# drtconway/zotmer

Hardware: AMD Instinct MI355X
Metric: Gk-mers/sec kmerize k=25 on synthetic 150bp FASTQ; achieved HBM GB/s fraction (higher is better)
Workload: dtype u64

## Files before the change

include/zotk.h:

```cpp
#ifndef ZOTK_H
#define ZOTK_H

#include <stdint.h>

#ifdef __cplusplus
extern "C" {
#endif

#define ZK_OK 0
#define ZK_EINVAL (-1)
#define ZK_ENOMEM (-2)
#define ZK_EHIP (-3)
#define ZK_ENOSPC (-4)
#define ZK_EOVERFLOW (-5)
#define ZK_EINTERNAL (-6)
#define ZK_ERANGE (-7)

typedef struct zk_ctx zk_ctx;

zk_ctx* zk_create(int device, uint64_t workspace_bytes);
void zk_destroy(zk_ctx* ctx);
const char* zk_last_error(zk_ctx* ctx);
int zk_set_stream(zk_ctx* ctx, void* hip_stream);
void* zk_get_stream(zk_ctx* ctx);
// ... 11 lines not shown
int zk_upload_async(zk_ctx* ctx, void* d_dst, const void* src, uint64_t bytes);

#define ZK_TUNE_SORT_VARIANT 1
#define ZK_TUNE_PAIRS_VARIANT 2
#define ZK_TUNE_SHORT_SORT 3
#define ZK_TUNE_XCD_GROUP 5
#define ZK_TUNE_SIDE_DIV 4
#define ZK_TUNE_EARLY_COLLAPSE 7
#define ZK_TUNE_PACKED_PAIRS 8
#define ZK_TUNE_WIDE_TILES 9
#define ZK_TUNE_STREAM_PASS 10
#define ZK_TUNE_STREAM_RANGES 11
#define ZK_TUNE_TAG_WORDS 12
#define ZK_TUNE_DEDUPE_VARIANT 13
#define ZK_TUNE_DEDUPE_LIMIT 14
#define ZK_TUNE_DEDUPE_BITS 15
#define ZK_TUNE_COMM_CHUNK 6
#define ZK_TUNE_TAG_PASS 17
#define ZK_TUNE_KWAY 18
#define ZK_TUNE_TILE_SORT 19
#define ZK_TUNE_STRAND_BLOCKS 20
#define ZK_TUNE_COMM_SELF_LOOP 16
int zk_tune(zk_ctx* ctx, int what, int value);

#define ZK_PROF_HIST_STREAM 1
#define ZK_PROF_HIST_ARRAY 2
#define ZK_PROF_PASS_STREAM 3
#define ZK_PROF_PASS_KEYS 4
#define ZK_PROF_PASS_PAIRS 5
#define ZK_PROF_RLE 6
#define ZK_PROF_UNION 7
#define ZK_PROF_SELECT 8
#define ZK_PROF_MIRROR 9
#define ZK_PROF_INTERSECT 10
#define ZK_PROF_COUNT_HIST 11
#define ZK_PROF_PASS_PACKED 12
#define ZK_PROF_SAMPLE 13
#define ZK_PROF_TILE_SORT 14
#define ZK_PROF_CAPTURE_HITS 15
#define ZK_PROF_PROJECT_SUM 16
#define ZK_PROF_SPECTRUM 17
int zk_debug_buffer(zk_ctx* ctx, void* d_buf);
int zk_profile(zk_ctx* ctx, int enable);
int zk_profile_read(zk_ctx* ctx, int tag, uint64_t* launches, double* total_ms, uint64_t* algorithmic_bytes);


// ... 172 lines not shown
```

zotmer_amd/csrc/context.hip:

```cpp
#include <stdarg.h>
#include <string.h>

#include "internal.hpp"
#include <vector>

namespace zk {

int fail(zk_ctx* c, int code, const char* fmt, ...) {
    char buf[512];
    va_list ap;
    va_start(ap, fmt);
    vsnprintf(buf, sizeof buf, fmt, ap);
    va_end(ap);
    if (c) c->last_error = buf;
    return code;
}

void arena_reset(zk_ctx* c) { c->arena_off = 0; }

int arena_alloc(zk_ctx* c, uint64_t bytes, void** p) {
    const uint64_t need = (bytes + 255) & ~255ull;
    if (c->arena_off + need > c->arena_size) {
        if (c->arena_off != 0)
            return fail(c, ZK_ENOMEM, "workspace too small: %llu bytes in use, %llu more needed, %llu reserved (call zk_reserve)",
// ... 273 lines not shown
    if (what == ZK_TUNE_PAIRS_VARIANT) { c->pairs_variant = value; return ZK_OK; }
    if (what == ZK_TUNE_SHORT_SORT) { c->short_sort = value; return ZK_OK; }
    if (what == ZK_TUNE_SIDE_DIV) { c->side_div = value; return ZK_OK; }
    if (what == ZK_TUNE_WIDE_TILES) { c->wide_tiles = value ? 1 : 0; return ZK_OK; }
    if (what == ZK_TUNE_PACKED_PAIRS) { c->packed_pairs = value ? 1 : 0; return ZK_OK; }
    if (what == ZK_TUNE_EARLY_COLLAPSE) { c->early_collapse = value < 0 ? 0 : (value > 3 ? 3 : value); return ZK_OK; }
    if (what == ZK_TUNE_COMM_SELF_LOOP) { c->comm_self_loop = value ? 1 : 0; return ZK_OK; }
    if (what == ZK_TUNE_COMM_CHUNK) { c->comm_chunk_bytes = value > 0 ? (uint64_t)value : 0; return ZK_OK; }
    if (what == ZK_TUNE_STREAM_PASS) {
#ifdef ZK_PHASES
        c->stream_pass = value < 0 ? 0 : value;
#else
        if (value < 0 || value > 3) return fail(c, ZK_EINVAL, "stream pass variant %d (0, 1, 2 or 3)", value);
        c->stream_pass = value;
#endif
        return ZK_OK;
    }
    if (what == ZK_TUNE_TAG_WORDS) { c->tag_words = value < 0 ? 0 : (value > 2 ? 2 : value); return ZK_OK; }
    if (what == ZK_TUNE_DEDUPE_VARIANT) { c->dedupe_variant = value < 0 ? -1 : (value & 3); return ZK_OK; }
    if (what == ZK_TUNE_KWAY) { c->kway = value < 0 ? 0 : (value > 2 ? 2 : value); return ZK_OK; }
    if (what == ZK_TUNE_TILE_SORT) { c->tile_sort = value ? 1 : 0; return ZK_OK; }
    if (what == ZK_TUNE_TAG_PASS) { c->tag_pass = value ? 1 : 0; return ZK_OK; }
    if (what == ZK_TUNE_DEDUPE_BITS) { c->dedupe_bits = value < 0 ? 0 : value; return ZK_OK; }
    if (what == ZK_TUNE_STRAND_BLOCKS) { c->strand_blocks = value < 0 ? 0 : (value > 3 ? 1 : value); return ZK_OK; }
    if (what == ZK_TUNE_DEDUPE_LIMIT) { c->dedupe_limit = value < 1 ? 1 : (value > 65536 ? 65536 : value); return ZK_OK; }
    if (what == ZK_TUNE_STREAM_RANGES) { c->stream_ranges = value < 0 ? 0 : (value > 4096 ? 4096 : value); return ZK_OK; }
    if (what == ZK_TUNE_XCD_GROUP) {
        if (value < 0 || value > 32 || (value & (value - 1))) return fail(c, ZK_EINVAL, "xcd group must be 0 or a power of two <= 32");
        c->xcd_group = value;
        return ZK_OK;
    }
    return fail(c, ZK_EINVAL, "unknown tuning knob %d", what);
}

int zk_debug_buffer(zk_ctx* c, void* d_buf) {
    if (!c) return ZK_EINVAL;
    enter(c);
    c->dbg = (u64*)d_buf;
    return ZK_OK;
}

int zk_profile(zk_ctx* c, int enable) {
    if (!c) return ZK_EINVAL;
    enter(c);
    ZK_HIP(c, hipStreamSynchronize(c->stream));
    for (auto& r : c->prof) { (void)hipEventDestroy(r.a); (void)hipEventDestroy(r.b); }
    c->prof.clear();
    c->profile = enable != 0;
    return ZK_OK;
}

int zk_profile_read(zk_ctx* c, int tag, uint64_t* launches, double* total_ms, uint64_t* total_bytes) {
    if (!c) return ZK_EINVAL;
    enter(c);
    ZK_HIP(c, hipStreamSynchronize(c->stream));
// ... 83 lines not shown
```

zotmer_amd/csrc/internal.hpp:

```cpp
#pragma once
#include <hip/hip_runtime.h>
#include <stdint.h>
#include <stdio.h>
#include <string>
#include <vector>

#include "../../include/zotk.h"
#include "common.hpp"

struct zk_ctx {
    int device = 0;
    hipStream_t stream = nullptr;
    bool own_stream = false;
    int num_cus = 256;
    int sort_variant = 3;
    int short_sort = 0;
    int packed_pairs = 1;
    int wide_tiles = 1;
    int early_collapse = 1;
    int side_div = 8;
    int pairs_variant = 7;
    int stream_pass = 1;
    int tag_words = 2;
    int dedupe_variant = 0;
    int dedupe_limit = 65536;
    int tag_pass = 0;
    int kway = 1;
    int tile_sort = 1;
    int dedupe_bits = 0;
    int strand_blocks = 1;
    int stream_ranges = 0;

    char* arena = nullptr;
    uint64_t arena_size = 0;
    uint64_t arena_off = 0;

    char* aux = nullptr;
    uint64_t aux_size = 0;

    u64* status = nullptr;
    uint64_t status_words = 0;
    unsigned short* part16 = nullptr;
    uint64_t part16_words = 0;
    u32 epoch = 0;
    u32* d_ticket = nullptr;
    u32* d_xticket = nullptr;
    int num_xcd = 1;
    int xcd_group = 0;
    u32 ticket_base = 0;

    u32* d_err = nullptr;
    u64* d_scalars = nullptr;
// ... 67 lines not shown
                   StreamTags* tags = nullptr; };
int sort_rbits(zk_ctx* c);
PassPlan sort_plan_upper(zk_ctx* c, int key_bits, int lo_bit);
struct MirrorHist { int passes; int shift[4]; int bits[4]; u64* raw; };
int sort_first_bits(zk_ctx* c, int key_bits, int lo_bit);
struct DedupeResult {
    uint64_t n_out = 0;
    uint32_t flags = 0;
    uint32_t n_big = 0;
    u64 *cuts = nullptr, *nwords = nullptr, *incl = nullptr, *big = nullptr, *work = nullptr;
    u32* sub = nullptr;
    uint32_t chunks = 0;
    int pack = 0;
    int tag_bits = 0;
    bool unsorted = false;
};
int dedupe_pass(zk_ctx* c, const u64* keys, uint64_t n, int key_bits, int b, int pack, u64* work, uint64_t cap, DedupeResult* r,
                uint64_t* n_in = nullptr, uint64_t max_chunks = 0, const u32* tags = nullptr, const u64* tag_cuts = nullptr,
                bool unsorted = false);
int dedupe_sort_blocks(zk_ctx* c, DedupeResult& r);
int expand_tags(zk_ctx* c, const u32* tags, const u64* cuts, uint32_t blocks, int tag_bits, u64* keys_out, uint64_t first_block = 0, uint64_t n_blocks = 0);
int dedupe_finish(zk_ctx* c, const DedupeResult& r, u64* out_k, u32* out_c, u64* out_m = nullptr, int K = 0, int gbases = 0,
                  u64** mirror_hist = nullptr, int* mirror_group_bits = nullptr, bool packed_out = false);
int sort_keys_upper_counted(zk_ctx* c, u64* keys, u64* alt, uint64_t n, int key_bits, int lo_bit, u64* counted, u64** result);
int strand_blocks(zk_ctx* c, const DedupeResult& r, u64* keys_buf, uint64_t buf_words, int K, u64* out_k, u32* out_c, uint64_t cap,
                  uint64_t* n_out);
int collapse_pass(zk_ctx* c, const u64* keys, uint64_t n, int shift, int bits, int pack, u64* out, uint64_t cap, uint64_t* n_out,
                  uint64_t max_tiles = 0);
int sort_stream(zk_ctx* c, const StreamSrc& src, u64* buf_a, u64* buf_b, uint64_t cap, uint64_t* n_keys,
                uint64_t acgt[4], u64** result);
struct StreamRows { u32* rows = nullptr; u64* offs = nullptr; u32 ranges = 0, radix = 0; u32* gcodes = nullptr; u16* gvalid = nullptr;
                    u32 strands = 1;
                    bool wide = false; };
int stream_hist(zk_ctx* c, const u8* stream, uint64_t n_bytes, int K, int mode, const PassPlan& plan, u64* ghist, u32 gstride,
                u64* d_acgt, u64* d_n, u64* rec_info, u64* sample, u32 sample_cap, int sample_shift, u64 sample_value, u32* sample_n,
                void* image_room, uint64_t image_room_bytes, StreamRows* out);
struct StreamPlanes { u16* dig; int shift, bits; };
int stream_pass0(zk_ctx* c, uint64_t n_bytes, int K, int mode, int shift, int bits, const u64* ghist0, const StreamRows& rows,
                 uint64_t first_nl, bool uniform, u64* kout, uint64_t n, int variant, const StreamPlanes* planes = nullptr);
int stream_pass1(zk_ctx* c, const u32* tags, const u16* dig, uint64_t n, const u64* ghist0, uint32_t radix0, int bits1, u32* tout, u64* cuts);
int tile_sort_top_bits(uint64_t n, int key_bits, int rbits);
int tile_sort(zk_ctx* c, u64* keys, u32* vals, uint64_t n, int key_bits, int top, bool* declined);
int tile_sort_count(zk_ctx* c, const u64* keys, uint64_t n, int key_bits, int top, u64* uniq, u32* counts, uint64_t cap, uint64_t* n_unique,
                    bool* declined);
int trim(zk_ctx* c, const u64* keys, const void* cnts, int cbits, uint64_t n, u64 lo, u64 hi, u64* ok, void* oc,
         uint64_t cap, uint64_t* n_out);
int project_dedupe(zk_ctx* c, const u64* keys, uint64_t n, int shift, u64* out, uint64_t cap, uint64_t* n_out);
// ... 45 lines not shown
```

zotmer_amd/csrc/pipeline.hip:

```cpp
#include <string.h>

#include <vector>

#include "internal.hpp"

namespace zk {

__global__ void mirror_kernel(const u64* __restrict__ c, const u32* __restrict__ n, u64 m, int K, u64* __restrict__ r,
                              u32* __restrict__ v) {
    for (u64 i = (u64)blockIdx.x * blockDim.x + threadIdx.x; i < m; i += (u64)gridDim.x * blockDim.x) {
        r[i] = revcomp(K, c[i]);
        v[i] = n[i];
    }
}

constexpr int MIRROR_GROUP_BITS = 18;
constexpr int MIRROR_GROUP_BASES = MIRROR_GROUP_BITS / 2;

__global__ void mirror_bounds_kernel(const u64* __restrict__ c, u64 n, int K, int gbits, u64* __restrict__ start) {
    const u32 g = blockIdx.x * blockDim.x + threadIdx.x;
    if (g > (1u << gbits)) return;
    const u64 want = (u64)g << (2 * K - gbits);
    u64 lo = 0, hi = n;
    if (g == (1u << gbits)) lo = n;
// ... 317 lines not shown
        st->n_canonical = 0;
        return rle(c, sorted, n, out_k, out_c, cap, n_out);
    }
    u64* other = (sorted == buf_a) ? buf_b : buf_a;
    u32* cnt = (u32*)other;
    uint64_t uc = 0;
    bool in_aux = false;
    uint64_t max_count = 0;
    bool have_max = false;
    bool canon_packed = false;
    u64 *mwords = nullptr, *malt = nullptr;
    u64* mhist = nullptr;
    int mgroup = MIRROR_GROUP_BITS;
    if (dedupe_bit && n) {
        const int pk = pack_bits_for(K);
        DedupeResult r;
        uint64_t n_in = 0;
        bool done = false;
        const uint64_t nblocks = 1ull << dedupe_bit, per = n / nblocks + 1;
        const u32* tg = stags.written ? (const u32*)sorted : nullptr;
        if (!presampled) ZK_TRY(dedupe_pass(c, sorted, n, 2 * K, dedupe_bit, pk, other, cap_keys, &r, &n_in, (1u << 20) / per + 4, tg, stags.cuts));
        if (presampled || (!(r.flags & 1) && (double)r.n_out <= 0.6 * (double)n_in)) {
            const bool route = !canonical_only && c->packed_pairs && dedupe_bit == MIRROR_GROUP_BITS && 2 * K >= MIRROR_GROUP_BITS + 8 &&
                               (K & 1) && (c->strand_blocks == 1 || c->strand_blocks == 3);
            ZK_TRY(dedupe_pass(c, sorted, n, 2 * K, dedupe_bit, pk, other, cap_keys, &r, nullptr, 0, tg, stags.cuts, route));
            if (!(r.flags & 1)) {
                uc = r.n_out;
                const uint64_t a8 = (8 * uc + 255) & ~255ull, a4 = (4 * uc + 255) & ~255ull;
                const bool want_m = !(r.flags & 2) && !canonical_only && c->packed_pairs && dedupe_bit == MIRROR_GROUP_BITS &&
                                    2 * K >= MIRROR_GROUP_BITS + 8;
                if (want_m && (K & 1) && c->strand_blocks && 2 * a8 <= 8 * cap_keys) {
                    st->n_canonical = uc;
                    return strand_blocks(c, r, sorted, cap_keys, K, out_k, out_c, cap, n_out);
                }
                if (r.unsorted) ZK_TRY(dedupe_sort_blocks(c, r));
                char* aux;
                ZK_TRY(aux_require(c, a8 + a4, &aux));
                ZK_TRY(dedupe_finish(c, r, (u64*)aux, (u32*)(aux + a8), want_m ? sorted : nullptr, K, MIRROR_GROUP_BASES, &mhist, &mgroup, want_m));
                if (want_m) { mwords = sorted; malt = other; canon_packed = true; }
                sorted = (u64*)aux; cnt = (u32*)(aux + a8);
                in_aux = true;
                if (!(r.flags & 2)) { max_count = (1ull << pk) - 1; have_max = true; }
                done = true;
            }
        }
        if (!done) {
            u64* res = nullptr;
// ... 320 lines not shown
```

zotmer_amd/csrc/radix_sort.hip:

```cpp
#include <stdlib.h>
#include "internal.hpp"
#include "encode_tile.hpp"
#include "dedupe.hpp"

namespace zk {

constexpr int MAX_RADIX = 1024;

enum { SRC_ARRAY = 0, SRC_STREAM = 1 };

template <int BLOCK_, int ITEMS_, int RBITS_, int ROUNDS_ = 1, int WPE_ = 1, int SEG_ = 32, bool PIPE_ = false>
struct Cfg {
    static constexpr int BLOCK = BLOCK_, ITEMS = ITEMS_, RBITS = RBITS_, ROUNDS = ROUNDS_, WPE = WPE_, SEG = SEG_;
    static constexpr bool PIPE = PIPE_;
    static_assert(SEG == 0 || (BLOCK * ITEMS < 32768 && (SEG & (SEG - 1)) == 0), "16-bit tile counts");
    static constexpr int TILE = BLOCK * ITEMS, RADIX = 1 << RBITS, NW = BLOCK / 64;
    static constexpr int EXCH = TILE / ROUNDS, IPR = ITEMS / ROUNDS;
    static_assert(ITEMS % ROUNDS == 0, "ROUNDS");
    static constexpr int DPT = (RADIX + BLOCK - 1) / BLOCK;
    static_assert(ITEMS % 2 == 0 && 2 * ITEMS < 256, "ITEMS");
    static_assert(64 * ITEMS < 65536, "per-wave ranks are 16-bit");
    static_assert(RADIX <= MAX_RADIX && RBITS * MAX_PASSES >= 64, "RBITS");
};

// ... 1131 lines not shown
template <class C, bool PAIRS = false>
struct PipeSmem {
    static constexpr bool IMG_FITS = sizeof(TileImage<C::TILE>) <= sizeof(u16) * C::NW * C::RADIX;
    static constexpr int IMG_WORDS = (int)(sizeof(u16) * C::NW * C::RADIX / 8);
    static constexpr int IMG_T = IMG_FITS ? (IMG_WORDS - 3) * 16 : 16;
    u64 exch[C::TILE];
    u32 exv[PAIRS ? C::TILE : 1];
    union {
        u16 cnt[C::NW][C::RADIX];
        TileImage<PipeSmem::IMG_T> img;
    };
    u32 digit_off[C::RADIX];
    u64 gbase[C::RADIX];
    u32 wsum[C::NW];
    u32 ticket;
    u32 total_live;
    u32 abort;
};

template <class C, int SRC, int VAR = 0>
__global__ __launch_bounds__(C::BLOCK, C::WPE) void pass_pipe_kernel(SortArgs a, u32 tiles) {
    constexpr int BLOCK = C::BLOCK, ITEMS = C::ITEMS, RADIX = C::RADIX, NW = C::NW, DPT = C::DPT, TILE = C::TILE;
    constexpr bool PAIRS = VAR == 5 || VAR == 6;
    constexpr bool ATOM = VAR == 3 || VAR == 4 || VAR == 6, TAGS = VAR == 2 || VAR == 3;
    static_assert(!PAIRS || SRC == SRC_ARRAY, "pairs come from arrays");
    static_assert(!ATOM || (SRC == SRC_ARRAY && NW >= 2), "the counters of the adds are the first two rows of the per-wave counters");
    static_assert(C::ROUNDS == 1, "the pipeline parks a whole tile in LDS");
    constexpr int NS = RADIX / 64;
    __shared__ PipeSmem<C, VAR == 5 || VAR == 6> sm;
    static_assert(SRC == SRC_ARRAY || PipeSmem<C>::IMG_FITS, "the tile image lives in the counter area");
    static_assert(SRC == SRC_ARRAY || (ITEMS == 16 && PipeSmem<C>::IMG_WORDS <= 2 * BLOCK), "stream source: 16 consecutive windows per thread");
    const int tid = threadIdx.x, lane = tid & 63, wave = __builtin_amdgcn_readfirstlane(tid >> 6);
    const u32 dmask = (1u << a.bits) - 1u;
    u16* mycnt = sm.cnt[wave];

    if (tid == 0) sm.abort = 0;
    u32* cnt32 = reinterpret_cast<u32*>(&sm.cnt[0][0]);
    if (ATOM && tid < RADIX) cnt32[tid] = 0;
    bool dirty = false;
    const u32 first = take_ticket(a.ticket, &sm.ticket) - a.ticket_base;
    if (first < (u32)NS) {
        constexpr int U = 32;
        __builtin_amdgcn_s_setprio(3);
        u64* carry = sm.exch;
        if (tid < 64) carry[tid] = 0;
        __syncthreads();
        const u64 tag = st_pack(ZK_ST_INCLUSIVE, a.epoch, 0);
// ... 413 lines not shown
    static int launch_pipe(zk_ctx* c, SortArgs a) {
      if constexpr (C::PIPE) {
        const u32 tiles = tiles_for(a, SRC);
        if (tiles == 0) return ZK_OK;
        u32 grid = (u32)c->num_cus * (sizeof(PipeSmem<C>) > 80 * 1024 ? 1 : 2);
        if (grid > tiles) grid = tiles;
        grid += C::RADIX / 64;
        ZK_TRY(lookback_begin(c, (uint64_t)tiles * C::RADIX, grid, &a.epoch, &a.ticket_base));
        ZK_TRY(part16_begin(c, (uint64_t)tiles * C::RADIX, &a.part));
        ZK_HIP(c, hipMemsetAsync(c->d_xticket, 0, 8 * 32 * sizeof(u32), c->stream));
        a.xticket = c->d_xticket;
        a.nx = (c->xcd_group > 0 && c->num_xcd == 8) ? 8u : 1u;
        a.glog = 0;
        while ((1 << (a.glog + 1)) <= c->xcd_group) a.glog++;
        a.status = c->status;
        a.ticket = c->d_ticket;
        a.err = c->d_err;
        a.dbg = c->dbg;
        a.dbg2 = c->dbg ? c->dbg + 8ull * tiles : nullptr;
        prof_begin(c, SRC == SRC_STREAM ? ZK_PROF_PASS_STREAM : (a.prof_tag ? a.prof_tag : ZK_PROF_PASS_KEYS),
                   SRC == SRC_STREAM ? a.n_bytes + 8 * a.n : (a.tags_out ? 12 : 16) * a.n);
        if (SRC == SRC_ARRAY && a.tags_out && a.straddle)
            hipLaunchKernelGGL((pass_pipe_kernel<C, SRC_ARRAY, 3>), dim3(grid), dim3(C::BLOCK), 0, c->stream, a, tiles);
        else if (SRC == SRC_ARRAY && a.straddle)
            hipLaunchKernelGGL((pass_pipe_kernel<C, SRC_ARRAY, 4>), dim3(grid), dim3(C::BLOCK), 0, c->stream, a, tiles);
        else if (SRC == SRC_ARRAY && a.tags_out)
            hipLaunchKernelGGL((pass_pipe_kernel<C, SRC_ARRAY, 2>), dim3(grid), dim3(C::BLOCK), 0, c->stream, a, tiles);
        else if (SRC == SRC_ARRAY && a.prof_tag == ZK_PROF_PASS_PACKED)
            hipLaunchKernelGGL((pass_pipe_kernel<C, SRC, 1>), dim3(grid), dim3(C::BLOCK), 0, c->stream, a, tiles);
        else
            hipLaunchKernelGGL((pass_pipe_kernel<C, SRC, 0>), dim3(grid), dim3(C::BLOCK), 0, c->stream, a, tiles);
        prof_end(c);
        ZK_HIP(c, hipGetLastError());
      }
      return ZK_OK;
    }
    static constexpr bool PIPE_PAIRS = C::PIPE && C::ITEMS <= 8;
    static int launch_pipe_pairs(zk_ctx* c, SortArgs a) {
      if constexpr (PIPE_PAIRS) {
        const u32 tiles = (u32)div_up(a.n, C::TILE);
        if (tiles == 0) return ZK_OK;
        u32 grid = (u32)c->num_cus * (sizeof(PipeSmem<C, true>) > 80 * 1024 ? 1 : 2);
        if (grid > tiles) grid = tiles;
        grid += C::RADIX / 64;
        ZK_TRY(lookback_begin(c, (uint64_t)tiles * C::RADIX, grid, &a.epoch, &a.ticket_base));
        ZK_TRY(part16_begin(c, (uint64_t)tiles * C::RADIX, &a.part));
        ZK_HIP(c, hipMemsetAsync(c->d_xticket, 0, 8 * 32 * sizeof(u32), c->stream));
        a.xticket = c->d_xticket;
        a.nx = 1u;
        a.glog = 0;
        a.status = c->status;
        a.ticket = c->d_ticket;
        a.err = c->d_err;
        a.dbg = nullptr; a.dbg2 = nullptr;
        prof_begin(c, ZK_PROF_PASS_PAIRS, 24 * a.n);
        if (a.straddle) hipLaunchKernelGGL((pass_pipe_kernel<C, SRC_ARRAY, 6>), dim3(grid), dim3(C::BLOCK), 0, c->stream, a, tiles);
        else hipLaunchKernelGGL((pass_pipe_kernel<C, SRC_ARRAY, 5>), dim3(grid), dim3(C::BLOCK), 0, c->stream, a, tiles);
        prof_end(c);
        ZK_HIP(c, hipGetLastError());
      }
      return ZK_OK;
    }
    static u32 keys_pass_tile(zk_ctx* c, uint64_t n) {
        if constexpr (C::PIPE && C::RBITS == 9 && C::BLOCK == 512) { if (c->wide_tiles && n <= WIDE_TILES_MAX_KEYS) return 16384u; }
        return (u32)C::TILE;
    }
    static int launch_keys_pass(zk_ctx* c, const SortArgs& a) {
        if constexpr (C::PIPE && C::RBITS == 9 && C::BLOCK == 512) { if (c->wide_tiles && a.n <= WIDE_TILES_MAX_KEYS) return launch_wide_pass(c, a); }
        if (C::PIPE) return launch_pipe<SRC_ARRAY>(c, a);
        return launch_pass<SRC_ARRAY, false>(c, a);
    }

    template <int SRC>
    static int launch_hist(zk_ctx* c, const SortArgs& src, const PassPlan& plan, u64* ghist, u64* acgt, u64* d_n,
                           u64* sample = nullptr, u32 sample_cap = 0, int sample_shift = 0, u64 sample_value = 0) {
        HistArgs h;
        h.sample = sample; h.sample_cap = sample_cap; h.sample_shift = sample_shift; h.sample_value = sample_value;
        h.sample_n = (u32*)(c->d_scalars + 23);
        if (sample) ZK_HIP(c, hipMemsetAsync(c->d_scalars + 23, 0, sizeof(u64), c->stream));
        h.src = src;
        h.plan = plan;
        h.ghist = ghist;
        h.acgt = acgt;
        h.tiles = tiles_for(src, SRC);
        h.rec_info = nullptr;
        ZK_HIP(c, hipMemsetAsync(ghist, 0, sizeof(u64) * MAX_PASSES * C::RADIX, c->stream));
        if (SRC == SRC_STREAM && src.n_bytes) {
            h.rec_info = c->d_scalars + 20;
            ZK_HIP(c, hipMemsetAsync(h.rec_info, 0, 3 * sizeof(u64), c->stream));
            hipLaunchKernelGGL(first_newline_kernel, dim3(1), dim3(256), 0, c->stream, src.stream, (u64)src.n_bytes, h.rec_info);
        }
        if (acgt) ZK_HIP(c, hipMemsetAsync(acgt, 0, sizeof(u64) * 4, c->stream));
        u32 grid = h.tiles < (u32)(c->num_cus * 8) ? h.tiles : (u32)(c->num_cus * 8);
        if (grid == 0) grid = 1;
        prof_begin(c, SRC == SRC_STREAM ? ZK_PROF_HIST_STREAM : ZK_PROF_HIST_ARRAY, SRC == SRC_STREAM ? src.n_bytes : 8 * src.n);
        if constexpr (SRC == SRC_STREAM && C::ITEMS == 16 && C::BLOCK <= 512) {
            if (src.mode != ZK_KEYS_BOTH) hipLaunchKernelGGL((hist_kernel<C, SRC, true>), dim3(grid), dim3(C::BLOCK), 0, c->stream, h);
            else hipLaunchKernelGGL((hist_kernel<C, SRC, false>), dim3(grid), dim3(C::BLOCK), 0, c->stream, h);
        } else {
            hipLaunchKernelGGL((hist_kernel<C, SRC, false>), dim3(grid), dim3(C::BLOCK), 0, c->stream, h);
        }
        prof_end(c);
        ZK_HIP(c, hipGetLastError());
        hipLaunchKernelGGL(hist_scan_kernel, dim3(1), dim3(256), 0, c->stream, ghist, plan.passes, (int)C::RADIX, d_n);
        ZK_HIP(c, hipGetLastError());
        return ZK_OK;
    }

    static int sort_keys(zk_ctx* c, u64* keys, u64* alt, uint64_t n, int key_bits, u64** result, int lo_bit = 0, int prof_tag = 0,
                         u64* counted = nullptr) {
        PassPlan plan = make_plan(key_bits - lo_bit, C::RBITS, lo_bit);
        u64* ghist = counted;
        if (!counted) ZK_TRY(arena_alloc(c, sizeof(u64) * MAX_PASSES * C::RADIX, (void**)&ghist));
        SortArgs a = {};
        a.kin = keys; a.n = n;
        a.prof_tag = prof_tag;
        if (counted) {
            hipLaunchKernelGGL(hist_scan_kernel, dim3(1), dim3(256), 0, c->stream, ghist, plan.passes, (int)C::RADIX, c->d_scalars + 8);
            ZK_HIP(c, hipGetLastError());
        } else {
            ZK_TRY(launch_hist<SRC_ARRAY>(c, a, plan, ghist, nullptr, c->d_scalars + 8));
        }
        u64* in = keys; u64* out = alt;
        for (int p = 0; p < plan.passes; p++) {
            a.kin = in; a.kout = out; a.shift = plan.shift[p]; a.bits = plan.bits[p];
            a.ghist = ghist + p * C::RADIX;
            ZK_TRY(launch_keys_pass(c, a));
            u64* t = in; in = out; out = t;
        }
        *result = in;
        return ZK_OK;
    }

    static int sort_pairs(zk_ctx* c, u64* keys, u64* alt, u32* vals, u32* valt, uint64_t n, int key_bits, u64** rk, u32** rv,
                          const u64* src_k = nullptr, const u32* src_v = nullptr, int mirror_K = 0, int lo_bit = 0, bool unordered = false) {
        PassPlan plan = make_plan(key_bits - lo_bit, C::RBITS, lo_bit);
        u64* ghist;
        ZK_TRY(arena_alloc(c, sizeof(u64) * MAX_PASSES * C::RADIX, (void**)&ghist));
        SortArgs a = {};
        a.kin = mirror_K ? src_k : keys; a.n = n; a.mirror_K = mirror_K;
        ZK_TRY(launch_hist<SRC_ARRAY>(c, a, plan, ghist, nullptr, c->d_scalars + 8));
        const u64* in = mirror_K ? src_k : keys; const u32* vi = mirror_K ? src_v : vals;
        u64* out = mirror_K ? keys : alt; u32* vo = mirror_K ? vals : valt;
        for (int p = 0; p < plan.passes; p++) {
            a.kin = in; a.kout = out; a.vin = vi; a.vout = vo; a.shift = plan.shift[p]; a.bits = plan.bits[p];
            a.ghist = ghist + p * C::RADIX;
            a.mirror_K = (p == 0) ? mirror_K : 0;
            if constexpr (PIPE_PAIRS) {
                a.straddle = nullptr;
                if (unordered && p <= 1) {
                    const u32 tiles = (u32)div_up(n, C::TILE);
                    u32* bm;
                    ZK_TRY(arena_alloc(c, sizeof(u32) * (tiles / 32 + 1), (void**)&bm));
                    ZK_HIP(c, hipMemsetAsync(bm, 0, sizeof(u32) * (tiles / 32 + 1), c->stream));
                    if (p == 1) {
                        hipLaunchKernelGGL(straddle_kernel, dim3((C::RADIX + 255) / 256), dim3(256), 0, c->stream, (const u64*)(ghist + (p - 1) * C::RADIX),
                                           1u << plan.bits[p - 1], (u32)C::TILE, bm);
                        ZK_HIP(c, hipGetLastError());
                    }
                    a.straddle = bm;
                }
                ZK_TRY(launch_pipe_pairs(c, a));
            } else
            ZK_TRY((launch_pass<SRC_ARRAY, true>(c, a)));
            in = out; vi = vo;
            out = (out == keys) ? alt : keys;
            vo = (vo == vals) ? valt : vals;
        }
        *rk = const_cast<u64*>(in); *rv = const_cast<u32*>(vi);
        return ZK_OK;
    }

    static int sort_stream(zk_ctx* c, const StreamSrc& src, u64* buf_a, u64* buf_b, uint64_t cap, uint64_t* n_keys,
                           uint64_t acgt[4], u64** result) {
        const int top = (src.hi_bit > 0 && src.hi_bit < 2 * src.K) ? src.hi_bit : 2 * src.K;
        PassPlan plan = make_plan(top - src.lo_bit, C::RBITS, src.lo_bit);
        u64* ghist;
        ZK_TRY(arena_alloc(c, sizeof(u64) * MAX_PASSES * C::RADIX, (void**)&ghist));
        SortArgs a = {};
        a.stream = src.stream; a.n_bytes = src.n_bytes; a.K = src.K; a.mode = src.mode;
        u64* d_acgt = c->d_scalars + 0;
        u64* d_n = c->d_scalars + 8;
// ... 74 lines not shown
                    const uint32_t cpr = (uint32_t)((W + 15) / 16);
                    const uint32_t rpt = (C::BLOCK / cpr) / 16 * 16;
                    if (rpt >= 16 && (uint64_t)rpt * rec / 16 + 3 <= (uint64_t)PipeSmem<C>::IMG_WORDS &&
                        (double)rpt * (double)W > 1.02 * (double)C::TILE * (double)W / (double)rec) {
                        a.rec = (u32)rec; a.rpt = rpt; a.cpr = cpr; a.wpr = (u32)W;
                        a.cpr_inv = (u32)(((1ull << 32) + cpr - 1) / cpr);
                    }
                }
            }
            if (src.mode != ZK_KEYS_BOTH) ZK_TRY(launch_pipe<SRC_STREAM>(c, a));
            else ZK_TRY((launch_pass<SRC_STREAM, false>(c, a)));
        } else {
            ZK_TRY((launch_pass<SRC_STREAM, false>(c, a)));
        }
        u64* in = buf_a; u64* out = buf_b;
        a.rec = 0;
        const bool tags = src.tags && C::PIPE && plan.passes == 2 && plan.shift[0] <= 32 && src.mode == ZK_KEYS_CANONICAL;
        for (int p = 1; p < plan.passes; p++) {
            a.kin = in; a.kout = out; a.shift = plan.shift[p]; a.bits = plan.bits[p];
            a.ghist = ghist + p * C::RADIX;
            a.tags_out = (tags && p == plan.passes - 1) ? 1 : 0;
            a.straddle = nullptr;
            if ((a.tags_out || p == 1) && c->tag_words >= 2 && C::PIPE) {
                const u32 tile = keys_pass_tile(c, n), tiles = (u32)div_up(n, tile);
                u32* bm;
                ZK_TRY(arena_alloc(c, sizeof(u32) * (tiles / 32 + 1), (void**)&bm));
                ZK_HIP(c, hipMemsetAsync(bm, 0, sizeof(u32) * (tiles / 32 + 1), c->stream));
                hipLaunchKernelGGL(straddle_kernel, dim3((C::RADIX + 255) / 256), dim3(256), 0, c->stream, (const u64*)(ghist + (p - 1) * C::RADIX),
                                   1u << plan.bits[p - 1], tile, bm);
                ZK_HIP(c, hipGetLastError());
                a.straddle = bm;
            }
#ifdef ZK_PHASES
            if (const char* e = getenv("ZK_LOCAL_PASS")) a.dbg_local = atoi(e);
#endif
            ZK_TRY(launch_keys_pass(c, a));
#ifdef ZK_PHASES
            if (a.dbg_local) { *n_keys = 0; return ZK_OK; }
#endif
            if (a.tags_out) {
                const u32 tile = keys_pass_tile(c, n), tiles = (u32)div_up(n, tile);
                const uint64_t blocks = 1ull << (plan.bits[0] + plan.bits[1]);
                u64* cuts;
                ZK_TRY(arena_alloc(c, sizeof(u64) * (blocks + 1), (void**)&cuts));
                hipLaunchKernelGGL(tag_cuts_kernel, dim3(1u << plan.bits[0]), dim3(512), 0, c->stream, (const u64*)in, (u64)n, (const u64*)ghist,
                                   (const u64*)(ghist + C::RADIX), (const u64*)c->status, (u32)C::RADIX, tile, tiles, plan.shift[1], plan.bits[1],
                                   plan.bits[0], cuts);
                ZK_HIP(c, hipGetLastError());
                src.tags->cuts = cuts; src.tags->blocks = (uint32_t)blocks; src.tags->written = true;
            }
            u64* t = in; in = out; out = t;
        }
        *result = in;
// ... 48 lines not shown

int sort_pairs(zk_ctx* c, u64* keys, u64* alt, u32* vals, u32* valt, uint64_t n, int key_bits, u64** rk, u32** rv) {
    *rk = keys; *rv = vals;
    if (n == 0) return ZK_OK;
    const int top = c->tile_sort ? tile_sort_top_bits(n, key_bits, sort_pairs_rbits(c)) : 0;
    if (top) {
        u64* k1 = nullptr; u32* v1 = nullptr;
        bool declined = false;
        ZK_TRY(sort_pairs_upper(c, keys, alt, vals, valt, n, key_bits, key_bits - top, &k1, &v1));
        ZK_TRY(tile_sort(c, k1, v1, n, key_bits, top, &declined));
        *rk = k1; *rv = v1;
        if (!declined) return ZK_OK;
        return sort_pairs_lsd(c, k1, k1 == keys ? alt : keys, v1, v1 == vals ? valt : vals, n, key_bits, rk, rv);
    }
    return sort_pairs_lsd(c, keys, alt, vals, valt, n, key_bits, rk, rv);
}

int sort_keys_upper(zk_ctx* c, u64* keys, u64* alt, uint64_t n, int key_bits, int lo_bit, u64** result, int prof_tag) {
    *result = keys;
    if (n == 0 || lo_bit >= key_bits) return ZK_OK;
    ZK_SORT_DISPATCH(c, sort_keys(c, keys, alt, n, key_bits, result, lo_bit, prof_tag));
}

int sort_keys_upper_counted(zk_ctx* c, u64* keys, u64* alt, uint64_t n, int key_bits, int lo_bit, u64* counted, u64** result) {
    *result = keys;
    if (n == 0 || lo_bit >= key_bits) return ZK_OK;
    return Sorter<V3>::sort_keys(c, keys, alt, n, key_bits, result, lo_bit, ZK_PROF_PASS_PACKED, counted);
}

int sort_pairs_upper(zk_ctx* c, u64* keys, u64* alt, u32* vals, u32* valt, uint64_t n, int key_bits, int lo_bit, u64** rk, u32** rv) {
    *rk = keys; *rv = vals;
    if (n == 0) return ZK_OK;
    if (c->pairs_variant == 7) return Sorter<V7>::sort_pairs(c, keys, alt, vals, valt, n, key_bits, rk, rv, nullptr, nullptr, 0, lo_bit);
    ZK_SORT_DISPATCH_V(c->pairs_variant, sort_pairs(c, keys, alt, vals, valt, n, key_bits, rk, rv, nullptr, nullptr, 0, lo_bit));
}

int sort_pairs_mirrored(zk_ctx* c, const u64* src_k, const u32* src_v, u64* keys, u64* alt, u32* vals, u32* valt, uint64_t n, int K,
                        u64** rk, u32** rv, int lo_bit) {
    *rk = keys; *rv = vals;
    if (n == 0) return ZK_OK;
    if (c->pairs_variant == 7) return Sorter<V7>::sort_pairs(c, keys, alt, vals, valt, n, 2 * K, rk, rv, src_k, src_v, K, lo_bit, true);
    ZK_SORT_DISPATCH_V(c->pairs_variant, sort_pairs(c, keys, alt, vals, valt, n, 2 * K, rk, rv, src_k, src_v, K, lo_bit));
}
int sort_pairs_rbits(zk_ctx* c) { return (c->pairs_variant == 0 || c->pairs_variant == 1 || c->pairs_variant == 5) ? 8 : 9; }

PassPlan sort_plan_upper(zk_ctx* c, int key_bits, int lo_bit) { return make_plan(key_bits - lo_bit, sort_rbits(c), lo_bit); }

int sort_rbits(zk_ctx* c) {
    switch (c->sort_variant) { case 0: case 1: case 5: return 8; default: return 9; }
}
// ... 208 lines not shown
```

zotmer_amd/csrc/strand_blocks.hip:

```cpp
#include "tile_group.hpp"

namespace zk {

constexpr int SB_ITEMS = 16, SB_GROUPS = 2048;
constexpr u32 SB_GROUP_MAX = 128;
typedef TileSortSmem<SB_ITEMS, SB_GROUPS, false> StrandSmem;
constexpr int SB_BLOCK_BITS = 18;

__global__ __launch_bounds__(256) void strand_mirror_kernel(const u64* __restrict__ in, const u64* __restrict__ cuts, const u64* __restrict__ incl,
                                                            const u64* __restrict__ nwords, u32 chunks, int pack, int K, u64* __restrict__ out_m,
                                                            MirrorHist mh) {
    __shared__ u32 bins[4 * 512];
    const bool hist = mh.passes > 0;
    if (hist) {
        for (int q = threadIdx.x; q < 4 * 512; q += blockDim.x) bins[q] = 0;
        __syncthreads();
    }
    const u64 maxc = (1ull << pack) - 1;
    for (u32 v = blockIdx.x; v < chunks; v += gridDim.x) {
        const u64 cnt = nwords[v];
        const u64 dst0 = incl[v] - cnt;
        const u64* src = in + cuts[v];
        for (u64 i0 = threadIdx.x; i0 < cnt; i0 += 4ull * blockDim.x) {
            u64 w4[4];
// ... 227 lines not shown
}

int dedupe_sort_blocks(zk_ctx* c, DedupeResult& r) {
    if (!r.unsorted || r.n_out == 0) { r.unsorted = false; return ZK_OK; }
    prof_begin(c, ZK_PROF_RLE, 16 * r.n_out);
    hipLaunchKernelGGL(dedupe_sort_blocks_kernel, dim3(r.chunks < (u32)c->num_cus ? r.chunks : (u32)c->num_cus), dim3(TS_BLOCK), 0, c->stream, r.work, r.cuts,
                       r.nwords, r.chunks, r.tag_bits + r.pack);
    prof_end(c);
    ZK_HIP(c, hipGetLastError());
    r.unsorted = false;
    return ZK_OK;
}

int strand_blocks(zk_ctx* c, const DedupeResult& r, u64* keys_buf, uint64_t buf_words, int K, u64* out_k, u32* out_c, uint64_t cap,
                  uint64_t* n_out) {
    *n_out = 0;
    const uint64_t uc = r.n_out;
    if (uc == 0) return ZK_OK;
    if (!(K & 1) || r.n_big || r.chunks != (1u << SB_BLOCK_BITS)) return fail(c, ZK_EINTERNAL, "strand_blocks: K %d, %u big counts, %u blocks", K, r.n_big, r.chunks);
    const uint64_t a8w = ((8 * uc + 255) & ~255ull) / 8;
    if (2 * a8w > buf_words) return fail(c, ZK_EINTERNAL, "strand_blocks: %llu words do not fit twice in %llu", (unsigned long long)uc, (unsigned long long)buf_words);
    if (2 * uc > cap) return fail(c, ZK_ENOSPC, "output holds %llu entries, the table has %llu", (unsigned long long)cap, (unsigned long long)(2 * uc));
    const int pk = r.pack, key_bits = 2 * K + pk, lo_bit = key_bits - SB_BLOCK_BITS;
    u64* mw = keys_buf;
    u64* malt = keys_buf + a8w;
    MirrorHist mh = {};
    if (c->sort_variant == 3) {
        const PassPlan plan = sort_plan_upper(c, key_bits, lo_bit);
        if (plan.passes <= 4) {
            ZK_TRY(arena_alloc(c, sizeof(u64) * MAX_PASSES * 512, (void**)&mh.raw));
            ZK_HIP(c, hipMemsetAsync(mh.raw, 0, sizeof(u64) * MAX_PASSES * 512, c->stream));
            mh.passes = plan.passes;
            for (int p = 0; p < plan.passes; p++) { mh.shift[p] = plan.shift[p]; mh.bits[p] = plan.bits[p]; }
        }
    }
    prof_begin(c, ZK_PROF_SELECT, 16 * uc);
    hipLaunchKernelGGL(strand_mirror_kernel, dim3((u32)c->num_cus * 8), dim3(256), 0, c->stream, r.work, r.cuts, r.incl, r.nwords, r.chunks, pk, K, mw, mh);
    prof_end(c);
    ZK_HIP(c, hipGetLastError());
    u64* sk = nullptr;
    if (mh.passes) ZK_TRY(sort_keys_upper_counted(c, mw, malt, uc, key_bits, lo_bit, mh.raw, &sk));
    else ZK_TRY(sort_keys_upper(c, mw, malt, uc, key_bits, lo_bit, &sk));
    u64* mstart;
    u32* declined;
    ZK_TRY(arena_alloc(c, sizeof(u64) * ((1ull << SB_BLOCK_BITS) + 1), (void**)&mstart));
    ZK_TRY(arena_alloc(c, sizeof(u32) * r.chunks, (void**)&declined));
    StrandArgs a = {};
    a.cw = r.work; a.cuts = r.cuts; a.nwords = r.nwords; a.incl = r.incl; a.m = sk; a.mstart = mstart;
    a.ok = out_k; a.oc = out_c; a.pack = pk; a.pshift = lo_bit;
    a.n_declined = (u32*)(c->d_scalars + 9);
    a.declined = declined;
    u32* fail = (u32*)(c->d_scalars + 9) + 1;
    prof_begin(c, ZK_PROF_UNION, 8 * 2 * uc + 12 * 2 * uc);
    hipLaunchKernelGGL(strand_starts_kernel, dim3(((1u << SB_BLOCK_BITS) + 256) / 256), dim3(256), 0, c->stream, sk, (u64)uc, lo_bit, mstart);
    ZK_HIP(c, hipMemsetAsync(c->d_scalars + 9, 0, sizeof(u64), c->stream));
    hipLaunchKernelGGL(strand_block_union_kernel, dim3(r.chunks), dim3(TS_BLOCK), 0, c->stream, a);
    prof_end(c);
    ZK_HIP(c, hipGetLastError());
    ZK_HIP(c, hipMemcpyAsync(c->h_scalars + 9, c->d_scalars + 9, sizeof(u64), hipMemcpyDeviceToHost, c->stream));
    ZK_TRY(check_device_error(c));
    const uint32_t n_declined = (uint32_t)c->h_scalars[9];
    if (n_declined && c->strand_blocks == 3) c->h_scalars[9] |= 1ull << 32;
    else if (n_declined) {
        const uint32_t grid = n_declined < 2u * (uint32_t)c->num_cus ? n_declined : 2u * (uint32_t)c->num_cus;
        u64* scratch;
        ZK_TRY(arena_alloc(c, sizeof(u64) * StrandSmem::CAP * grid, (void**)&scratch));
        prof_begin(c, ZK_PROF_UNION, 0);
        hipLaunchKernelGGL(strand_big_block_kernel, dim3(grid), dim3(TS_BLOCK), 0, c->stream, a, n_declined, scratch, fail);
        prof_end(c);
        ZK_HIP(c, hipGetLastError());
        ZK_HIP(c, hipMemcpyAsync(c->h_scalars + 9, c->d_scalars + 9, sizeof(u64), hipMemcpyDeviceToHost, c->stream));
        ZK_TRY(check_device_error(c));
    }
    if ((uint32_t)(c->h_scalars[9] >> 32) == 0) {
        *n_out = 2 * uc;
        return ZK_OK;
    }
    DedupeResult rs = r;
    ZK_TRY(dedupe_sort_blocks(c, rs));
    char* aux;
    ZK_TRY(aux_require(c, 8 * a8w, &aux));
    ZK_TRY(dedupe_finish(c, rs, (u64*)aux, nullptr, nullptr, K, 0, nullptr, nullptr, true));
    u64* ms = nullptr;
    ZK_TRY(sort_keys_upper(c, sk, sk == mw ? malt : mw, uc, key_bits, pk, &ms));
    return union_sum_packed_ab(c, (const u64*)aux, uc, ms, uc, pk, out_k, out_c, cap, n_out, true);
}

}
```

zotmer_amd/native.py:

```python
import ctypes as C
import os

import numpy as np

_HERE = os.path.dirname(os.path.abspath(__file__))
LIB_PATH = os.environ.get("ZOTK_LIB") or os.path.join(_HERE, "libzotk.so")

ZK_OK, ZK_EINVAL, ZK_ENOMEM, ZK_EHIP, ZK_ENOSPC, ZK_EOVERFLOW, ZK_EINTERNAL, ZK_ERANGE = 0, -1, -2, -3, -4, -5, -6, -7
KMERIZE_CANONICAL, KMERIZE_BOTH, KMERIZE_SUBSAMPLE, KMERIZE_CANONICAL_ONLY = 0, 1, 2, 4
DEFAULT_TAG_WORDS = 2

_ERRNAMES = {-1: "ZK_EINVAL", -2: "ZK_ENOMEM", -3: "ZK_EHIP", -4: "ZK_ENOSPC", -5: "ZK_EOVERFLOW",
             -6: "ZK_EINTERNAL", -7: "ZK_ERANGE"}


class ZotkError(RuntimeError):
    def __init__(self, code, msg):
        super().__init__("%s: %s" % (_ERRNAMES.get(code, code), msg))
        self.code = code


class Spectrum(C.Structure):
    _fields_ = [("n_shared", C.c_uint64), ("s_min", C.c_uint64), ("x_shared", C.c_uint64), ("y_shared", C.c_uint64),
                ("s_xy_lo", C.c_uint64), ("s_xy_hi", C.c_uint64), ("s_sqrt", C.c_double), ("s_js", C.c_double)]
# ... 8 lines not shown
_pu64 = C.POINTER(C.c_uint64)
SIGNATURES = {
    "zk_create": (_vp, [_i, _u64]),
    "zk_destroy": (None, [_vp]),
    "zk_last_error": (C.c_char_p, [_vp]),
    "zk_set_stream": (_i, [_vp, _vp]),
    "zk_get_stream": (_vp, [_vp]),
    "zk_sync": (_i, [_vp]),
    "zk_reserve": (_i, [_vp, _u64]),
    "zk_release_workspace": (_i, [_vp]),
    "zk_mem_info": (_i, [_vp, _pu64, _pu64]),
    "zk_alloc": (_i, [_vp, _u64, C.POINTER(_vp)]),
    "zk_free": (_i, [_vp, _vp]),
    "zk_upload": (_i, [_vp, _vp, _vp, _u64]),
    "zk_download": (_i, [_vp, _vp, _vp, _u64]),
    "zk_copy": (_i, [_vp, _vp, _vp, _u64]),
    "zk_host_alloc": (_i, [_vp, _u64, C.POINTER(_vp)]),
    "zk_host_free": (_i, [_vp, _vp]),
    "zk_upload_async": (_i, [_vp, _vp, _vp, _u64]),
    "zk_tune": (_i, [_vp, _i, _i]),
    "zk_debug_buffer": (_i, [_vp, _vp]),
    "zk_profile": (_i, [_vp, _i]),
    "zk_profile_read": (_i, [_vp, _i, _pu64, C.POINTER(C.c_double), _pu64]),
    "zk_pack_reads": (_i, [_vp, _vp, _vp, _u64, _vp]),
    "zk_encode": (_i, [_vp, _vp, _u64, _i, _i, _vp, _u64, _pu64, _pu64]),
    "zk_capture_filter": (_i, [_vp, _vp, _u64, _i, _vp, _u64, _vp, _pu64, _pu64]),
    "zk_subsample": (_i, [_vp, _vp, _u64, _u64, _d, _vp, _u64, _pu64]),
    "zk_can": (_i, [_vp, _i, _vp, _u64, _vp]),
    "zk_sort_keys": (_i, [_vp, _vp, _u64, _i]),
    "zk_sort_pairs": (_i, [_vp, _vp, _vp, _u64, _i]),
    "zk_rle": (_i, [_vp, _vp, _u64, _vp, _vp, _u64, _pu64]),
    "zk_sort_count": (_i, [_vp, _vp, _u64, _i, _vp, _vp, _u64, _pu64]),
    "zk_kmerize": (_i, [_vp, _vp, _u64, _i, _i, _d, _u64, _vp, _vp, _u64, C.POINTER(KmerizeStats)]),
    "zk_mirror_expand": (_i, [_vp, _vp, _vp, _u64, _i, _vp, _vp, _u64, _pu64]),
    "zk_hist": (_i, [_vp, _vp, _i, _u64, _pu64, _pu64, _u64, _pu64]),
    "zk_widen_counts": (_i, [_vp, _vp, _vp, _u64]),
    "zk_union_sum": (_i, [_vp, _vp, _vp, _u64, _vp, _vp, _u64, _vp, _vp, _i, _u64, _pu64, _pu64]),
    "zk_merge_n": (_i, [_vp, _i, C.POINTER(_vp), C.POINTER(_vp), _pu64, _vp, _vp, _i, _u64, _pu64, _pu64]),
    "zk_project_dedupe": (_i, [_vp, _vp, _u64, _i, _vp, _u64, _pu64]),
    "zk_project": (_i, [_vp, _vp, _u64, _vp, _vp, _u64, _vp, _vp, _u64, _pu64]),
    "zk_sample": (_i, [_vp, _vp, _vp, _u64, _u64, _d, _vp, _vp, _u64, _pu64]),
    "zk_split": (_i, [_vp, _vp, _u64, _vp, _u64, _pu64]),
    "zk_project_sum": (_i, [_vp, _vp, _vp, _i, _u64, _i, _vp, _vp, _u64, _pu64, _pu64]),
    "zk_spectrum_sums": (_i, [_vp, _vp, _vp, _u64, _vp, _vp, _u64, _d, _d, C.POINTER(Spectrum)]),
    "zk_lower_bound": (_i, [_vp, _vp, _u64, _pu64, _u32, _pu64]),
    "zk_trim": (_i, [_vp, _vp, _vp, _i, _u64, _u64, _u64, _vp, _vp, _u64, _pu64]),
# ... 283 lines not shown
        if xcd_group is not None:
            self._check(self.lib.zk_tune(self.h, 5, int(xcd_group)))
        if short_sort is not None:
            self._check(self.lib.zk_tune(self.h, 3, int(short_sort)))
        if side_div is not None:
            self._check(self.lib.zk_tune(self.h, 4, int(side_div)))
        if sort_variant is not None:
            self._check(self.lib.zk_tune(self.h, 1, int(sort_variant)))
        if pairs_variant is not None:
            self._check(self.lib.zk_tune(self.h, 2, int(pairs_variant)))

    def profile(self, enable=True):
        self._check(self.lib.zk_profile(self.h, int(enable)))

    def profile_read(self):
        out = {}
        for name, tag in self.PROF_TAGS.items():
            n, b, ms = C.c_uint64(0), C.c_uint64(0), C.c_double(0)
            self._check(self.lib.zk_profile_read(self.h, tag, C.byref(n), C.byref(ms), C.byref(b)))
            if n.value:
                out[name] = dict(launches=n.value, ms=ms.value, bytes=b.value)
        return out

    def pack_reads(self, bases, offs):
        n_reads = offs.n - 1
        total = int(offs.to_host()[-1]) if offs.n else 0
        out = self.empty(total + n_reads, np.uint8)
        self._check(self.lib.zk_pack_reads(self.h, bases.ptr, offs.ptr, n_reads, out.ptr))
        return out

    def encode(self, stream, K, both=True):
        cap = stream.n * (2 if both else 1)
        out = self.empty(cap, np.uint64)
        n = C.c_uint64(0)
        acgt = (C.c_uint64 * 4)()
        self._check(self.lib.zk_encode(self.h, stream.ptr, stream.n, K, int(both), out.ptr, cap, C.byref(n), acgt))
        return out.view(n.value), [int(v) for v in acgt]

    def subsample(self, kmers, seed, p):
        out = self.empty(kmers.n, np.uint64)
        n = C.c_uint64(0)
        self._check(self.lib.zk_subsample(self.h, kmers.ptr, kmers.n, int(seed), float(p), out.ptr, kmers.n, C.byref(n)))
        return out.view(n.value)

    def can(self, K, kmers):
        out = self.empty(kmers.n, np.uint64)
# ... 353 lines not shown
```

Baseline: 163.0.

## Use atomic unordered scatter passes in strand-block upper sort

When strand blocks mode is 1 or 3 (default 1), the upper-bits key sort in strand_blocks now runs its first two passes in unordered mode. These passes get straddle bitmaps and a new pass-pipe variant 7 that uses atomic ranking instead of ordered per-tile offsets. This should cut the inter-tile ordering and sync cost, since later dedupe tolerates unordered keys within buckets. It also factors out a shared straddle-bitmap helper, adds route counters with a query API, and adds mode 4, which takes the routing path but not the unordered sort.

```diff
diff --git a/include/zotk.h b/include/zotk.h
--- a/include/zotk.h
+++ b/include/zotk.h
@@ -57,6 +57,7 @@
 #define ZK_TUNE_STRAND_BLOCKS 20
 #define ZK_TUNE_COMM_SELF_LOOP 16
 int zk_tune(zk_ctx* ctx, int what, int value);
+int zk_route_stats(zk_ctx* ctx, uint64_t stats[4]);
 
 #define ZK_PROF_HIST_STREAM 1
 #define ZK_PROF_HIST_ARRAY 2
diff --git a/zotmer_amd/csrc/context.hip b/zotmer_amd/csrc/context.hip
--- a/zotmer_amd/csrc/context.hip
+++ b/zotmer_amd/csrc/context.hip
@@ -319,7 +319,7 @@
     if (what == ZK_TUNE_TILE_SORT) { c->tile_sort = value ? 1 : 0; return ZK_OK; }
     if (what == ZK_TUNE_TAG_PASS) { c->tag_pass = value ? 1 : 0; return ZK_OK; }
     if (what == ZK_TUNE_DEDUPE_BITS) { c->dedupe_bits = value < 0 ? 0 : value; return ZK_OK; }
-    if (what == ZK_TUNE_STRAND_BLOCKS) { c->strand_blocks = value < 0 ? 0 : (value > 3 ? 1 : value); return ZK_OK; }
+    if (what == ZK_TUNE_STRAND_BLOCKS) { c->strand_blocks = value < 0 ? 0 : (value > 4 ? 1 : value); return ZK_OK; }
     if (what == ZK_TUNE_DEDUPE_LIMIT) { c->dedupe_limit = value < 1 ? 1 : (value > 65536 ? 65536 : value); return ZK_OK; }
     if (what == ZK_TUNE_STREAM_RANGES) { c->stream_ranges = value < 0 ? 0 : (value > 4096 ? 4096 : value); return ZK_OK; }
     if (what == ZK_TUNE_XCD_GROUP) {
@@ -328,6 +328,13 @@
         return ZK_OK;
     }
     return fail(c, ZK_EINVAL, "unknown tuning knob %d", what);
+}
+
+int zk_route_stats(zk_ctx* c, uint64_t stats[4]) {
+    if (!c || !stats) return ZK_EINVAL;
+    enter(c);
+    for (int i = 0; i < 4; i++) stats[i] = c->route_stats[i];
+    return ZK_OK;
 }
 
 int zk_debug_buffer(zk_ctx* c, void* d_buf) {
diff --git a/zotmer_amd/csrc/internal.hpp b/zotmer_amd/csrc/internal.hpp
--- a/zotmer_amd/csrc/internal.hpp
+++ b/zotmer_amd/csrc/internal.hpp
@@ -28,6 +28,7 @@
     int kway = 1;
     int tile_sort = 1;
     int dedupe_bits = 0;
+    uint64_t route_stats[4] = {0, 0, 0, 0};
     int strand_blocks = 1;
     int stream_ranges = 0;
 
@@ -141,7 +142,7 @@
 int expand_tags(zk_ctx* c, const u32* tags, const u64* cuts, uint32_t blocks, int tag_bits, u64* keys_out, uint64_t first_block = 0, uint64_t n_blocks = 0);
 int dedupe_finish(zk_ctx* c, const DedupeResult& r, u64* out_k, u32* out_c, u64* out_m = nullptr, int K = 0, int gbases = 0,
                   u64** mirror_hist = nullptr, int* mirror_group_bits = nullptr, bool packed_out = false);
-int sort_keys_upper_counted(zk_ctx* c, u64* keys, u64* alt, uint64_t n, int key_bits, int lo_bit, u64* counted, u64** result);
+int sort_keys_upper_counted(zk_ctx* c, u64* keys, u64* alt, uint64_t n, int key_bits, int lo_bit, u64* counted, u64** result, bool unordered = false);
 int strand_blocks(zk_ctx* c, const DedupeResult& r, u64* keys_buf, uint64_t buf_words, int K, u64* out_k, u32* out_c, uint64_t cap,
                   uint64_t* n_out);
 int collapse_pass(zk_ctx* c, const u64* keys, uint64_t n, int shift, int bits, int pack, u64* out, uint64_t cap, uint64_t* n_out,
diff --git a/zotmer_amd/csrc/pipeline.hip b/zotmer_amd/csrc/pipeline.hip
--- a/zotmer_amd/csrc/pipeline.hip
+++ b/zotmer_amd/csrc/pipeline.hip
@@ -363,7 +363,7 @@
         if (!presampled) ZK_TRY(dedupe_pass(c, sorted, n, 2 * K, dedupe_bit, pk, other, cap_keys, &r, &n_in, (1u << 20) / per + 4, tg, stags.cuts));
         if (presampled || (!(r.flags & 1) && (double)r.n_out <= 0.6 * (double)n_in)) {
             const bool route = !canonical_only && c->packed_pairs && dedupe_bit == MIRROR_GROUP_BITS && 2 * K >= MIRROR_GROUP_BITS + 8 &&
-                               (K & 1) && (c->strand_blocks == 1 || c->strand_blocks == 3);
+                               (K & 1) && (c->strand_blocks == 1 || c->strand_blocks == 3 || c->strand_blocks == 4);
             ZK_TRY(dedupe_pass(c, sorted, n, 2 * K, dedupe_bit, pk, other, cap_keys, &r, nullptr, 0, tg, stags.cuts, route));
             if (!(r.flags & 1)) {
                 uc = r.n_out;
diff --git a/zotmer_amd/csrc/radix_sort.hip b/zotmer_amd/csrc/radix_sort.hip
--- a/zotmer_amd/csrc/radix_sort.hip
+++ b/zotmer_amd/csrc/radix_sort.hip
@@ -1177,7 +1177,7 @@
 __global__ __launch_bounds__(C::BLOCK, C::WPE) void pass_pipe_kernel(SortArgs a, u32 tiles) {
     constexpr int BLOCK = C::BLOCK, ITEMS = C::ITEMS, RADIX = C::RADIX, NW = C::NW, DPT = C::DPT, TILE = C::TILE;
     constexpr bool PAIRS = VAR == 5 || VAR == 6;
-    constexpr bool ATOM = VAR == 3 || VAR == 4 || VAR == 6, TAGS = VAR == 2 || VAR == 3;
+    constexpr bool ATOM = VAR == 3 || VAR == 4 || VAR == 6 || VAR == 7, TAGS = VAR == 2 || VAR == 3;
     static_assert(!PAIRS || SRC == SRC_ARRAY, "pairs come from arrays");
     static_assert(!ATOM || (SRC == SRC_ARRAY && NW >= 2), "the counters of the adds are the first two rows of the per-wave counters");
     static_assert(C::ROUNDS == 1, "the pipeline parks a whole tile in LDS");
@@ -1637,6 +1637,8 @@
                    SRC == SRC_STREAM ? a.n_bytes + 8 * a.n : (a.tags_out ? 12 : 16) * a.n);
         if (SRC == SRC_ARRAY && a.tags_out && a.straddle)
             hipLaunchKernelGGL((pass_pipe_kernel<C, SRC_ARRAY, 3>), dim3(grid), dim3(C::BLOCK), 0, c->stream, a, tiles);
+        else if (SRC == SRC_ARRAY && a.straddle && a.prof_tag == ZK_PROF_PASS_PACKED)
+            hipLaunchKernelGGL((pass_pipe_kernel<C, SRC_ARRAY, 7>), dim3(grid), dim3(C::BLOCK), 0, c->stream, a, tiles);
         else if (SRC == SRC_ARRAY && a.straddle)
             hipLaunchKernelGGL((pass_pipe_kernel<C, SRC_ARRAY, 4>), dim3(grid), dim3(C::BLOCK), 0, c->stream, a, tiles);
         else if (SRC == SRC_ARRAY && a.tags_out)
@@ -1680,6 +1682,16 @@
         if constexpr (C::PIPE && C::RBITS == 9 && C::BLOCK == 512) { if (c->wide_tiles && n <= WIDE_TILES_MAX_KEYS) return 16384u; }
         return (u32)C::TILE;
     }
+    static int straddle_bitmap(zk_ctx* c, uint64_t n, u32 tile, const u64* starts, u32 buckets, u32** bitmap) {
+        const u32 tiles = (u32)div_up(n, tile);
+        ZK_TRY(arena_alloc(c, sizeof(u32) * (tiles / 32 + 1), (void**)bitmap));
+        ZK_HIP(c, hipMemsetAsync(*bitmap, 0, sizeof(u32) * (tiles / 32 + 1), c->stream));
+        if (starts) {
+            hipLaunchKernelGGL(straddle_kernel, dim3((C::RADIX + 255) / 256), dim3(256), 0, c->stream, starts, buckets, tile, *bitmap);
+            ZK_HIP(c, hipGetLastError());
+        }
+        return ZK_OK;
+    }
     static int launch_keys_pass(zk_ctx* c, const SortArgs& a) {
         if constexpr (C::PIPE && C::RBITS == 9 && C::BLOCK == 512) { if (c->wide_tiles && a.n <= WIDE_TILES_MAX_KEYS) return launch_wide_pass(c, a); }
         if (C::PIPE) return launch_pipe<SRC_ARRAY>(c, a);
@@ -1723,7 +1735,7 @@
     }
 
     static int sort_keys(zk_ctx* c, u64* keys, u64* alt, uint64_t n, int key_bits, u64** result, int lo_bit = 0, int prof_tag = 0,
-                         u64* counted = nullptr) {
+                         u64* counted = nullptr, bool unordered = false) {
         PassPlan plan = make_plan(key_bits - lo_bit, C::RBITS, lo_bit);
         u64* ghist = counted;
         if (!counted) ZK_TRY(arena_alloc(c, sizeof(u64) * MAX_PASSES * C::RADIX, (void**)&ghist));
@@ -1740,6 +1752,15 @@
         for (int p = 0; p < plan.passes; p++) {
             a.kin = in; a.kout = out; a.shift = plan.shift[p]; a.bits = plan.bits[p];
             a.ghist = ghist + p * C::RADIX;
+            a.straddle = nullptr;
+            if constexpr (C::PIPE) {
+                if (unordered && p <= 1) {
+                    u32* bm;
+                    ZK_TRY(straddle_bitmap(c, n, keys_pass_tile(c, n), p == 1 ? ghist : nullptr, 1u << plan.bits[0], &bm));
+                    a.straddle = bm;
+                    c->route_stats[2]++;
+                }
+            }
             ZK_TRY(launch_keys_pass(c, a));
             u64* t = in; in = out; out = t;
         }
@@ -1764,15 +1785,8 @@
             if constexpr (PIPE_PAIRS) {
                 a.straddle = nullptr;
                 if (unordered && p <= 1) {
-                    const u32 tiles = (u32)div_up(n, C::TILE);
                     u32* bm;
-                    ZK_TRY(arena_alloc(c, sizeof(u32) * (tiles / 32 + 1), (void**)&bm));
-                    ZK_HIP(c, hipMemsetAsync(bm, 0, sizeof(u32) * (tiles / 32 + 1), c->stream));
-                    if (p == 1) {
-                        hipLaunchKernelGGL(straddle_kernel, dim3((C::RADIX + 255) / 256), dim3(256), 0, c->stream, (const u64*)(ghist + (p - 1) * C::RADIX),
-                                           1u << plan.bits[p - 1], (u32)C::TILE, bm);
-                        ZK_HIP(c, hipGetLastError());
-                    }
+                    ZK_TRY(straddle_bitmap(c, n, (u32)C::TILE, p == 1 ? ghist : nullptr, 1u << plan.bits[0], &bm));
                     a.straddle = bm;
                 }
                 ZK_TRY(launch_pipe_pairs(c, a));
@@ -1893,13 +1907,8 @@
             a.tags_out = (tags && p == plan.passes - 1) ? 1 : 0;
             a.straddle = nullptr;
             if ((a.tags_out || p == 1) && c->tag_words >= 2 && C::PIPE) {
-                const u32 tile = keys_pass_tile(c, n), tiles = (u32)div_up(n, tile);
                 u32* bm;
-                ZK_TRY(arena_alloc(c, sizeof(u32) * (tiles / 32 + 1), (void**)&bm));
-                ZK_HIP(c, hipMemsetAsync(bm, 0, sizeof(u32) * (tiles / 32 + 1), c->stream));
-                hipLaunchKernelGGL(straddle_kernel, dim3((C::RADIX + 255) / 256), dim3(256), 0, c->stream, (const u64*)(ghist + (p - 1) * C::RADIX),
-                                   1u << plan.bits[p - 1], tile, bm);
-                ZK_HIP(c, hipGetLastError());
+                ZK_TRY(straddle_bitmap(c, n, keys_pass_tile(c, n), ghist + (p - 1) * C::RADIX, 1u << plan.bits[p - 1], &bm));
                 a.straddle = bm;
             }
 #ifdef ZK_PHASES
@@ -1994,10 +2003,10 @@
     ZK_SORT_DISPATCH(c, sort_keys(c, keys, alt, n, key_bits, result, lo_bit, prof_tag));
 }
 
-int sort_keys_upper_counted(zk_ctx* c, u64* keys, u64* alt, uint64_t n, int key_bits, int lo_bit, u64* counted, u64** result) {
+int sort_keys_upper_counted(zk_ctx* c, u64* keys, u64* alt, uint64_t n, int key_bits, int lo_bit, u64* counted, u64** result, bool unordered) {
     *result = keys;
     if (n == 0 || lo_bit >= key_bits) return ZK_OK;
-    return Sorter<V3>::sort_keys(c, keys, alt, n, key_bits, result, lo_bit, ZK_PROF_PASS_PACKED, counted);
+    return Sorter<V3>::sort_keys(c, keys, alt, n, key_bits, result, lo_bit, ZK_PROF_PASS_PACKED, counted, unordered);
 }
 
 int sort_pairs_upper(zk_ctx* c, u64* keys, u64* alt, u32* vals, u32* valt, uint64_t n, int key_bits, int lo_bit, u64** rk, u32** rv) {
diff --git a/zotmer_amd/csrc/strand_blocks.hip b/zotmer_amd/csrc/strand_blocks.hip
--- a/zotmer_amd/csrc/strand_blocks.hip
+++ b/zotmer_amd/csrc/strand_blocks.hip
@@ -273,6 +273,7 @@
     if (2 * a8w > buf_words) return fail(c, ZK_EINTERNAL, "strand_blocks: %llu words do not fit twice in %llu", (unsigned long long)uc, (unsigned long long)buf_words);
     if (2 * uc > cap) return fail(c, ZK_ENOSPC, "output holds %llu entries, the table has %llu", (unsigned long long)cap, (unsigned long long)(2 * uc));
     const int pk = r.pack, key_bits = 2 * K + pk, lo_bit = key_bits - SB_BLOCK_BITS;
+    c->route_stats[0]++;
     u64* mw = keys_buf;
     u64* malt = keys_buf + a8w;
     MirrorHist mh = {};
@@ -290,7 +291,7 @@
     prof_end(c);
     ZK_HIP(c, hipGetLastError());
     u64* sk = nullptr;
-    if (mh.passes) ZK_TRY(sort_keys_upper_counted(c, mw, malt, uc, key_bits, lo_bit, mh.raw, &sk));
+    if (mh.passes) ZK_TRY(sort_keys_upper_counted(c, mw, malt, uc, key_bits, lo_bit, mh.raw, &sk, c->strand_blocks == 1 || c->strand_blocks == 3));
     else ZK_TRY(sort_keys_upper(c, mw, malt, uc, key_bits, lo_bit, &sk));
     u64* mstart;
     u32* declined;
@@ -327,6 +328,7 @@
         *n_out = 2 * uc;
         return ZK_OK;
     }
+    c->route_stats[1]++;
     DedupeResult rs = r;
     ZK_TRY(dedupe_sort_blocks(c, rs));
     char* aux;
diff --git a/zotmer_amd/native.py b/zotmer_amd/native.py
--- a/zotmer_amd/native.py
+++ b/zotmer_amd/native.py
@@ -54,6 +54,7 @@
     "zk_debug_buffer": (_i, [_vp, _vp]),
     "zk_profile": (_i, [_vp, _i]),
     "zk_profile_read": (_i, [_vp, _i, _pu64, C.POINTER(C.c_double), _pu64]),
+    "zk_route_stats": (_i, [_vp, _pu64]),
     "zk_pack_reads": (_i, [_vp, _vp, _vp, _u64, _vp]),
     "zk_encode": (_i, [_vp, _vp, _u64, _i, _i, _vp, _u64, _pu64, _pu64]),
     "zk_capture_filter": (_i, [_vp, _vp, _u64, _i, _vp, _u64, _vp, _pu64, _pu64]),
@@ -383,6 +384,11 @@
                 out[name] = dict(launches=n.value, ms=ms.value, bytes=b.value)
         return out
 
+    def route_stats(self):
+        s = (C.c_uint64 * 4)()
+        self._check(self.lib.zk_route_stats(self.h, s))
+        return dict(strand_route=int(s[0]), strand_other_way=int(s[1]), add_ranked_passes=int(s[2]))
+
     def pack_reads(self, bases, offs):
         n_reads = offs.n - 1
         total = int(offs.to_host()[-1]) if offs.n else 0
```

Result: no change. 164.1, median of 6 (+0.7%).
